# RazonIn4K/image-restoration-platform

Measured on AMD Instinct MI355X. Metric: restored images/sec @1024x1024 bs=8, higher is better.
Workload: dtype bf16; 1 GPU; 1024x1024 RGB u8, batch 8 per GPU: fused classifier scan + RestoreNet-v0 (43 convs, 779.9 GFLOP/image), seeded random-init weights; global_batch=8, parallelism=per-image data parallel x1, no collective, streams=1

## Files before the change

image_restoration_platform_amd/csrc/conv_pc.hip:

```cpp
#include "conv_mfma.hpp"
#include "conv_plan.hpp"
#include "gn_fold.hpp"
#include "persist.hpp"

#include <type_traits>

namespace ire {

namespace {

typedef __bf16 bf16x8_t __attribute__((ext_vector_type(8)));
typedef __bf16 bf16x2_t __attribute__((ext_vector_type(2)));
typedef float f32x2_t __attribute__((ext_vector_type(2)));
typedef float f32x16_t __attribute__((ext_vector_type(16)));
typedef unsigned u32x4_t __attribute__((ext_vector_type(4)));

#ifndef C3_RES_PRE
#define C3_RES_PRE -1
#endif
#ifndef C3_SCALAR
#define C3_SCALAR 1
#endif
#ifndef C3_PRIO
#define C3_PRIO 1
#endif
#ifndef C3_TEPI
#define C3_TEPI 1
#endif
#ifndef IRE_LD_ONCE32
#define IRE_LD_ONCE32 2
#endif
#ifndef C3_TEPI64
#define C3_TEPI64 1
#endif
#ifndef C3_PROD8
#define C3_PROD8 0
#endif
#ifndef C3_INTERIOR
#define C3_INTERIOR 0
#endif
#ifndef C3_ABL
#define C3_ABL 0
#endif
constexpr int C3_CONS = 512, C3_PROD = 256, C3_THREADS = C3_CONS + C3_PROD;
constexpr int pc_prod(int C, bool head) { return (C3_PROD8 && C == 32 && !head) ? 512 : 256; }
constexpr int C3_TH = 16, C3_TW = 32, C3_IH = C3_TH + 2, C3_IW = C3_TW + 2;
constexpr int C3_IN_CHUNKS = C3_IH * C3_IW * 4;
constexpr int C3_P_ITERS = (C3_IN_CHUNKS + C3_PROD - 1) / C3_PROD;
constexpr int C3_IN_BYTES = C3_P_ITERS * C3_PROD * 16;
template <int C> struct PcCfg {
    static constexpr int NT = C < 64 ? 32 : 64;
    static constexpr int NBLK = C / NT;
    static constexpr int NKC = C / 32;
    static constexpr int NTL = NT / 32;
    static constexpr int W_STAGE = 36 * NT * 16;
    static constexpr int W_STAGE_CHUNKS = 36 * NT;
    static constexpr int W_LDS = NKC * W_STAGE;
    static constexpr int W_OFF = 2 * C3_IN_BYTES;
    static constexpr int BIAS_OFF = W_OFF + W_LDS;
    static constexpr int NCC = NT / 8;
    static constexpr int RED_OFF = BIAS_OFF + C * 4;
    static constexpr int RED_HALF = 8 * NCC * 4;
    static constexpr int COEF_IMGS = pc_coef_imgs(C);
    static constexpr int COEF_OFF = RED_OFF + 2 * RED_HALF * 4;
    static constexpr int HEAD_OFF = COEF_OFF + COEF_IMGS * C * 2 * 4;
    static constexpr int PATCH_OFF = HEAD_OFF + (C == 32 ? 8 * 2 * 2 * 96 : 0);
    static constexpr int CNT_OFF = PATCH_OFF + (C == 32 ? 8 * 2048 : 0);
    static constexpr int LDS = CNT_OFF + (C == 64 ? 16 : 0);
    static_assert(LDS <= 160 * 1024, "LDS");
};

__device__ __forceinline__ unsigned c3_pack(float a, float b) {
    f32x2_t f = {a, b};
    return __builtin_bit_cast(unsigned, __builtin_convertvector(f, bf16x2_t));
}
__device__ __forceinline__ float c3_lo(unsigned u) { return __builtin_bit_cast(float, u << 16); }
__device__ __forceinline__ float c3_hi(unsigned u) { return __builtin_bit_cast(float, u & 0xffff0000u); }
template <int N> __device__ __forceinline__ float c3_ror_add(float v) {
    const int r = __builtin_amdgcn_update_dpp(0, __builtin_bit_cast(int, v), 0x120 + N, 0xf, 0xf, false);
    return v + __builtin_bit_cast(float, r);
}
__device__ __forceinline__ float c3_swap16_add(float v) {
    float x = v, y = v;
    asm volatile("v_nop\n\tv_nop\n\tv_permlane16_swap_b32 %0, %1" : "+v"(x), "+v"(y));
    return x + y;
}

__device__ __forceinline__ void c3_glds16(const void* gsrc, unsigned lds_dst_uniform) {
    unsigned keep;
    asm volatile("s_mov_b32 %0, m0\n\ts_mov_b32 m0, %2\n\ts_nop 0\n\tglobal_load_lds_dwordx4 %1, off\n\ts_mov_b32 m0, %0"
                 : "=&s"(keep) : "v"(gsrc), "s"(lds_dst_uniform) : "memory");
}
__device__ __forceinline__ void c3_barrier() { asm volatile("s_waitcnt lgkmcnt(0)\n\ts_barrier" ::: "memory"); }

template <int C, bool RESID, bool HEAD>
__global__ __launch_bounds__(C3_CONS + pc_prod(C, HEAD)) void conv_pc_kernel(ConvArgs a) {
    using K = PcCfg<C>;
    constexpr int PROD = pc_prod(C, HEAD), THREADS = C3_CONS + PROD;
    constexpr int P_ITERS = (C3_IN_CHUNKS + PROD - 1) / PROD;
    static_assert(P_ITERS * PROD * 16 == C3_IN_BYTES, "tile slots");
    constexpr int NKC = K::NKC, NTL = K::NTL, NCC = K::NCC, NT = K::NT;
    static_assert(!HEAD || C == 32, "the head is a C = 32 layer");
    __shared__ __attribute__((aligned(16))) unsigned char smem[K::LDS];
    const int tid = threadIdx.x;
    const int lane = tid & 63, wave = tid >> 6;
    const int r = lane & 31, h = lane >> 5;
    int stamp_item = 0;
    auto stamp = [&](int k) {
#ifdef IRE_PC_TICKS
        const unsigned long long t = __builtin_amdgcn_s_memtime();
        if (a.stamps && lane == 0 && (wave == 0 || wave == 8) && blockIdx.x < 8 && stamp_item < 64)
            a.stamps[(((size_t)blockIdx.x * 2 + (wave ? 1 : 0)) * 64 + stamp_item) * 10 + k] = t;
#else
        (void)k;
#endif
    };

    auto tl = [&](int slot) {
#ifdef IRE_W4_TL
        if (a.stamps && tid == 0) {
            a.stamps[(size_t)blockIdx.x * 32 + slot * 2] = __builtin_amdgcn_s_memrealtime();
            a.stamps[(size_t)blockIdx.x * 32 + slot * 2 + 1] = __builtin_amdgcn_s_memtime();
        }
#else
        (void)slot;
#endif
    };
    const int tiles_per_img = a.tiles_x * a.tiles_y;
    PersistCursor cursor(a.tiles_x, a.tiles_y, a.nimg, K::NBLK, NKC, (int)gridDim.x, (int)blockIdx.x, a.walk_rev != 0);
    const int n_items = cursor.my_items;
    if (n_items == 0) return;
    const int n_stages = n_items * NKC;
    tl(0);
    {
        const unsigned char* ws = reinterpret_cast<const unsigned char*>(a.w);
        const unsigned wl = (unsigned)(size_t)(__attribute__((address_space(3))) unsigned char*)smem + K::W_OFF;
        constexpr int PIECES = NKC * K::W_STAGE_CHUNKS / 64;
        static_assert((NKC * K::W_STAGE_CHUNKS) % 64 == 0, "whole wave-instructions");
        const int wv = __builtin_amdgcn_readfirstlane(wave);
        for (int p = wv; p < PIECES; p += THREADS / 64) c3_glds16(ws + ((size_t)p * 64 + lane) * 16, wl + p * 1024);
    }
    if (a.gn_stats) gn_fold(a, smem, cursor.first_img, cursor.last_img, 512, reinterpret_cast<float2*>(smem + K::COEF_OFF));
    tl(1);

    {
        if (tid < C) reinterpret_cast<float*>(smem + K::BIAS_OFF)[tid] = a.bias[tid];
        if constexpr (C == 64) { if (tid == 0) *reinterpret_cast<unsigned*>(smem + K::CNT_OFF) = 0u; }
        const int nim = cursor.last_img - cursor.first_img + 1;
        const float2* ab = a.ab + (size_t)cursor.first_img * C;
        float2* cd = reinterpret_cast<float2*>(smem + K::COEF_OFF);
        if (!a.gn_stats) for (int i = tid; i < nim * C; i += THREADS) cd[i] = ab[i];
    }
    asm volatile("s_waitcnt vmcnt(0)" ::: "memory");
    __syncthreads();
    tl(2);

    if (__builtin_amdgcn_readfirstlane(wave) >= 8) {
#if C3_PRIO
        if (C3_PRIO != 1 || C != 32 || HEAD) asm volatile("s_setprio %0" :: "n"(C3_PRIO));
#endif
        const int tp = tid - C3_CONS;
        const int c8 = tp & 3;
        int rel[P_ITERS], lds_off[P_ITERS];
        unsigned pyx[P_ITERS];
#pragma unroll
        for (int i = 0; i < P_ITERS; ++i) {
            const int q = tp + i * PROD;
            const int p = q >> 2;
            const int py = p / C3_IW, px = p - py * C3_IW;
            pyx[i] = ((unsigned)py << 8) | (unsigned)px;
            rel[i] = (py * a.Win + px) * (2 * C) + c8 * 16;
            lds_off[i] = (p * 4 + (c8 ^ ((p >> 2) & 3))) * 16;
        }
        uint4 R[P_ITERS];
        unsigned okbits = 0;
        float cA[8], cB[8];
        PersistStage ls = cursor.cur;
        auto load_chunk = [&](int i) __attribute__((always_inline)) {
            const PersistItem& lit = ls.it;
            const int oy1 = lit.ty * C3_TH - 1, ox1 = lit.tx * C3_TW - 1;
            const char* base = reinterpret_cast<const char*>(a.in0) + (size_t)lit.img * a.in_rows * a.Win * (2 * C) + ls.kc * 64;
            const __amdgpu_buffer_rsrc_t irsrc = __builtin_amdgcn_make_buffer_rsrc(const_cast<char*>(base), 0, a.in_rows * a.Win * (2 * C) - ls.kc * 64, 0x00020000);
            const int base_off = ((oy1 + a.in_row_off) * a.Win + ox1) * (2 * C);
            const int y_lo = max(a.iy_lo - oy1, 0), y_hi = min(a.iy_lo + a.iy_span - oy1, C3_IH);
            const int x_lo = max(-ox1, 0), x_hi = min(a.Win - ox1, C3_IW);
            const int py = (int)(pyx[i] >> 8), px = (int)(pyx[i] & 0xffu);
            const bool ok = (unsigned)(py - y_lo) < (unsigned)(y_hi - y_lo) && (unsigned)(px - x_lo) < (unsigned)(x_hi - x_lo);
            const unsigned off = ok ? (unsigned)(base_off + rel[i]) : 0xffffffffu;
            if constexpr (C3_ABL & 8) { R[i] = make_uint4(off, 0x3f803f80u, i, 0x3f803f80u); }
            else {
                const u32x4_t lv = __builtin_amdgcn_raw_buffer_load_b128(irsrc, off, 0, IRE_LD_IN);
                R[i] = make_uint4(lv.x, lv.y, lv.z, lv.w);
            }
            okbits = (okbits & ~(1u << i)) | (ok ? (1u << i) : 0u);
        };
        auto load_coeffs = [&](const PersistStage& st) __attribute__((always_inline)) {
            const float4* ab = reinterpret_cast<const float4*>(smem + K::COEF_OFF) + ((st.it.img - cursor.first_img) * C + st.kc * 32 + c8 * 8) / 2;
#pragma unroll
            for (int e = 0; e < 4; ++e) { const float4 v = ab[e]; cA[2 * e] = v.x; cB[2 * e] = v.y; cA[2 * e + 1] = v.z; cB[2 * e + 1] = v.w; }
        };
        auto transform_stage_v = [&](unsigned char* tile, auto interior_tag) __attribute__((always_inline)) {
            constexpr bool INTERIOR = decltype(interior_tag)::value;
            auto pair = [&](auto pp_tag) __attribute__((always_inline)) {
                constexpr int pp_ = decltype(pp_tag)::value, i = 2 * pp_;
                constexpr int NCH = i + 1 < P_ITERS ? 2 : 1;
                constexpr int NW = 4 * NCH, NV = 8 * NCH;
                constexpr int i1 = NCH == 2 ? i + 1 : i;
                const unsigned wds[8] = {R[i].x, R[i].y, R[i].z, R[i].w, R[i1].x, R[i1].y, R[i1].z, R[i1].w};
                unsigned o[8];
                if constexpr (C3_ABL & 1) {
#pragma unroll
                    for (int w = 0; w < NW; ++w) o[w] = wds[w];
                } else {
#if C3_SCALAR
                    float y[16], e[16];
#pragma unroll
                    for (int w = 0; w < NW; ++w) {
                        const int d = w & 3;
                        y[2 * w] = __builtin_fmaf(c3_lo(wds[w]), cA[2 * d], cB[2 * d]);
                        y[2 * w + 1] = __builtin_fmaf(c3_hi(wds[w]), cA[2 * d + 1], cB[2 * d + 1]);
                    }
#pragma unroll
                    for (int k = 0; k < NV; ++k) e[k] = y[k] * (-1.4426950408889634f);
                    __builtin_amdgcn_sched_barrier(0);
#pragma unroll
                    for (int k = 0; k < NV; ++k) e[k] = __builtin_amdgcn_exp2f(e[k]);
                    __builtin_amdgcn_sched_barrier(0);
#pragma unroll
                    for (int k = 0; k < NV; ++k) e[k] = e[k] + 1.0f;
                    __builtin_amdgcn_sched_barrier(0);
#pragma unroll
                    for (int k = 0; k < NV; ++k) e[k] = __builtin_amdgcn_rcpf(e[k]);
                    __builtin_amdgcn_sched_barrier(0);
#pragma unroll
                    for (int w = 0; w < NW; ++w) o[w] = c3_pack(y[2 * w] * e[2 * w], y[2 * w + 1] * e[2 * w + 1]);
#else
                    static_assert(NCH == 2, "the packed-f32 form handles whole pairs");
                    f32x2_t y[8], e[8];
#pragma unroll
                    for (int w = 0; w < 8; ++w) {
                        const int d = w & 3;
                        const f32x2_t x = {c3_lo(wds[w]), c3_hi(wds[w])};
                        const f32x2_t A = {cA[2 * d], cA[2 * d + 1]}, B = {cB[2 * d], cB[2 * d + 1]};
                        y[w] = __builtin_elementwise_fma(x, A, B);
                        e[w] = y[w] * (-1.4426950408889634f);
                    }
                    __builtin_amdgcn_sched_barrier(0);
#pragma unroll
                    for (int w = 0; w < 8; ++w) e[w] = f32x2_t{__builtin_amdgcn_exp2f(e[w].x), __builtin_amdgcn_exp2f(e[w].y)};
                    __builtin_amdgcn_sched_barrier(0);
#pragma unroll
                    for (int w = 0; w < 8; ++w) e[w] = e[w] + 1.0f;
                    __builtin_amdgcn_sched_barrier(0);
#pragma unroll
                    for (int w = 0; w < 8; ++w) e[w] = f32x2_t{__builtin_amdgcn_rcpf(e[w].x), __builtin_amdgcn_rcpf(e[w].y)};
                    __builtin_amdgcn_sched_barrier(0);
#pragma unroll
                    for (int w = 0; w < 8; ++w) { const f32x2_t sv = y[w] * e[w]; o[w] = c3_pack(sv.x, sv.y); }
#endif
                }
#pragma unroll
                for (int k = 0; k < NCH; ++k) {
                    uint4 ov = make_uint4(o[4 * k], o[4 * k + 1], o[4 * k + 2], o[4 * k + 3]);
                    if constexpr (!INTERIOR) {
                        const unsigned m = (okbits >> (i + k)) & 1u ? 0xffffffffu : 0u;
                        ov = make_uint4(o[4 * k] & m, o[4 * k + 1] & m, o[4 * k + 2] & m, o[4 * k + 3] & m);
                    }
                    *reinterpret_cast<uint4*>(tile + lds_off[i + k]) = ov;
                }
                load_chunk(i);
                if constexpr (NCH == 2) load_chunk(i + 1);
                __builtin_amdgcn_sched_barrier(0);
            };
            pair(std::integral_constant<int, 0>{}); pair(std::integral_constant<int, 1>{}); pair(std::integral_constant<int, 2>{});
            if constexpr (P_ITERS > 6) { pair(std::integral_constant<int, 3>{}); pair(std::integral_constant<int, 4>{}); }
        };
        unsigned past_last = 0u;
        {
            const int q = tp + (P_ITERS - 1) * PROD;
            past_last = (q >> 2) >= C3_IH * C3_IW ? (1u << (P_ITERS - 1)) : 0u;
        }
        auto transform_stage = [&](unsigned char* tile) __attribute__((always_inline)) {
            if constexpr (C3_INTERIOR) {
                if (__builtin_amdgcn_ballot_w64((okbits | past_last) != (1u << P_ITERS) - 1u) == 0) { transform_stage_v(tile, std::true_type{}); return; }
            }
            transform_stage_v(tile, std::false_type{});
        };
#pragma unroll
        for (int i = 0; i < P_ITERS; ++i) load_chunk(i);
        load_coeffs(ls);
        ls = cursor.next();
        transform_stage(smem);
        c3_barrier();
        for (int t = 0; t < n_stages; ++t) {
            stamp_item = t / NKC;
            stamp(3 * (t % NKC) + 0);
            load_coeffs(ls);
            ls = cursor.next();
            transform_stage(smem + ((t + 1) & 1) * C3_IN_BYTES);
            stamp(3 * (t % NKC) + 1);
            c3_barrier();
            stamp(3 * (t % NKC) + 2);
        }
        return;
    }

    int a_off[2][9];
#pragma unroll
    for (int m = 0; m < 2; ++m)
#pragma unroll
        for (int tap = 0; tap < 9; ++tap) {
            const int ky = tap / 3, kx = tap - ky * 3;
            const int p = (wave * 2 + m + ky) * C3_IW + r + kx;
            a_off[m][tap] = (p * 4 + (h ^ ((p >> 2) & 3))) * 16;
        }
    const unsigned char* wb = smem + K::W_OFF + (h * NT + r) * 16;
    const float* bias_lds = reinterpret_cast<const float*>(smem + K::BIAS_OFF);
    f32x16_t bias_acc;
    if constexpr (C == 32) {
#pragma unroll
        for (int i = 0; i < 16; ++i) bias_acc[i] = bias_lds[16 * (i >> 3) + 8 * h + (i & 7)];
    }
    float* red_base = reinterpret_cast<float*>(smem + K::RED_OFF);
    int st_img = -1, st_tile = 0, st_nb = 0, st_par = 0, red_par = 0;
    auto flush_stats = [&]() {
        if (HEAD || st_img < 0) return;
        constexpr int G = C / 8, NGL = NT / G, CPG = G / 8;
        if (tid < NGL) {
            const float* red = red_base + st_par * K::RED_HALF;
            float s = 0.f, q = 0.f;
#pragma unroll
            for (int w = 0; w < 8; ++w) {
                if constexpr (C == 32) {
                    const float* d = red + (w * NCC + (tid >> 1)) * 4 + 2 * (tid & 1);
                    s += d[0]; q += d[1];
                } else {
#pragma unroll
                    for (int k = 0; k < CPG; ++k) {
                        const float* d = red + (w * NCC + tid * CPG + k) * 4;
                        s += d[0] + d[2]; q += d[1] + d[3];
                    }
                }
            }
            float* st = a.stats + (((size_t)st_img * tiles_per_img + st_tile) * 8 + (st_nb * NT) / G + tid) * 2;
            st[0] = s; st[1] = q;
        }
        st_img = -1;
    };

    f32x16_t acc[2][NTL];
    uint4 erv[2 * NTL][2];
    constexpr int RES_WANT = C3_RES_PRE >= 0 ? C3_RES_PRE : (C == 64 ? 1 : 2);
    constexpr int RES_PRE = RES_WANT < 2 * NTL ? RES_WANT : 2 * NTL;
    unsigned eoffs[2];
    bool einb[2];
    constexpr bool TEPI = C3_TEPI && C == 32 && !HEAD;
    constexpr bool TEPI64 = C3_TEPI64 && C == 64 && !HEAD;
    unsigned toffs[2];
    bool trow[2];
    int tcol = 0;
    unsigned hin[2] = {0u, 0u};
    size_t hoff[2] = {0, 0};
    bool hok[2] = {false, false};
    PersistStage cs = cursor.cur;
    int stage_no = 0;
    c3_barrier();
    for (int t = 0; t < n_items; ++t) {
        const PersistItem it = cs.it;
        stamp_item = t;
        stamp(0);
        flush_stats();
        {
            const int oyb = it.ty * C3_TH + wave * 2, ox = it.tx * C3_TW + r;
            const bool colok = ox < a.Wout;
            const int oxc = min(ox, a.Wout - 1);
#pragma unroll
            for (int m = 0; m < 2; ++m) {
                const int oy = oyb + m;
                einb[m] = colok && oy < a.Hout;
                eoffs[m] = ((unsigned)((min(oy, a.Hout - 1) * a.Wout + oxc) * C + it.nb * NT) << 1) + (unsigned)(h * 16);
            }
            if constexpr (TEPI || TEPI64) {
                constexpr int LPP = C / 8;
                tcol = it.tx * C3_TW + lane / LPP;
#pragma unroll
                for (int m = 0; m < 2; ++m) {
                    const int oy = oyb + m;
                    trow[m] = oy < a.Hout;
                    toffs[m] = ((unsigned)((min(oy, a.Hout - 1) * a.Wout + tcol) * C + 8 * (lane % LPP)) << 1);
                }
            }
            if constexpr (RESID && TEPI64 && !(C3_ABL & 64)) {
                char* rbase = const_cast<char*>(reinterpret_cast<const char*>(a.resid)) + (size_t)it.img * a.Hout * a.Wout * (2 * C);
                const __amdgpu_buffer_rsrc_t rrsrc = __builtin_amdgcn_make_buffer_rsrc(rbase, 0, a.Hout * a.Wout * (2 * C), 0x00020000);
#pragma unroll
                for (int m = 0; m < 2; ++m)
#pragma unroll
                    for (int k = 0; k < RES_PRE; ++k) {
                        const bool ok = trow[m] && tcol + 8 * k < a.Wout;
                        const u32x4_t v = __builtin_amdgcn_raw_buffer_load_b128(rrsrc, ok ? toffs[m] + (unsigned)(8 * k * 2 * C) : 0xffffffffu, 0, IRE_LD_ONCE32);
                        erv[k][m] = make_uint4(v.x, v.y, v.z, v.w);
                    }
            } else
            if constexpr (RESID && TEPI && !(C3_ABL & 64)) {
                char* rbase = const_cast<char*>(reinterpret_cast<const char*>(a.resid)) + (size_t)it.img * a.Hout * a.Wout * (2 * C);
                const __amdgpu_buffer_rsrc_t rrsrc = __builtin_amdgcn_make_buffer_rsrc(rbase, 0, a.Hout * a.Wout * (2 * C), 0x00020000);
#pragma unroll
                for (int m = 0; m < 2; ++m)
#pragma unroll
                    for (int k = 0; k < 2; ++k) {
                        const bool ok = trow[m] && tcol + 16 * k < a.Wout;
                        const u32x4_t v = __builtin_amdgcn_raw_buffer_load_b128(rrsrc, ok ? toffs[m] + (unsigned)(16 * k * 2 * C) : 0xffffffffu, 0, IRE_LD_ONCE);
                        erv[k][m] = make_uint4(v.x, v.y, v.z, v.w);
                    }
            } else if constexpr (RESID && (C3_ABL & 64)) {
#pragma unroll
                for (int g = 0; g < 2 * NTL; ++g)
#pragma unroll
                    for (int m = 0; m < 2; ++m) erv[g][m] = make_uint4(eoffs[m], g, 0x3f803f80u, m);
            } else if constexpr (RESID) {
                const char* rbase = reinterpret_cast<const char*>(a.resid) + (size_t)it.img * a.Hout * a.Wout * (2 * C);
#pragma unroll
                for (int m = 0; m < 2; ++m)
#pragma unroll
                    for (int g = 0; g < RES_PRE; ++g) erv[g][m] = *reinterpret_cast<const uint4*>(rbase + eoffs[m] + (unsigned)(g * 32));
            }
            if constexpr (HEAD) {
                const int vbytes = 3 * min(C3_TW, a.Wout - it.tx * C3_TW);
#pragma unroll
                for (int m = 0; m < 2; ++m) {
                    const int oy = oyb + m;
                    hok[m] = oy < a.Hout && 4 * lane < vbytes;
                    hoff[m] = (((size_t)it.img * a.Hout + min(oy, a.Hout - 1)) * a.Wout + it.tx * C3_TW) * 3 + 4 * (size_t)min(lane, 23);
                    hin[m] = hok[m] ? *reinterpret_cast<const unsigned*>(a.u8_in + hoff[m]) : 0u;
                }
            }
        }
        if constexpr (C != 32) {
#pragma unroll
            for (int j = 0; j < NTL; ++j)
#pragma unroll
                for (int q = 0; q < 4; ++q) {
                    const float4 bv = *reinterpret_cast<const float4*>(bias_lds + it.nb * NT + j * 32 + 16 * (q >> 1) + 8 * h + 4 * (q & 1));
#pragma unroll
                    for (int m = 0; m < 2; ++m) { acc[m][j][4 * q + 0] = bv.x; acc[m][j][4 * q + 1] = bv.y; acc[m][j][4 * q + 2] = bv.z; acc[m][j][4 * q + 3] = bv.w; }
                }
        }
#pragma unroll NKC <= 2 ? NKC : 1
        for (int kc = 0; kc < NKC; ++kc) {
          auto stage_body = [&](auto par_tag) __attribute__((always_inline)) {
            constexpr int PAR = decltype(par_tag)::value;
            const int par = PAR >= 0 ? PAR : (stage_no & 1);
            const unsigned char* ib = smem + par * C3_IN_BYTES;
            const unsigned char* wk = wb + kc * K::W_STAGE;
            bf16x8_t af[2][2], bf[2][NTL];
            auto read_k = [&](int g, bf16x8_t (&pa)[2], bf16x8_t (&pw)[NTL]) __attribute__((always_inline)) {
                const int tap = g >> 1, cp = g & 1;
#pragma unroll
                for (int m = 0; m < 2; ++m) pa[m] = __builtin_bit_cast(bf16x8_t, *reinterpret_cast<const uint4*>(ib + (a_off[m][tap] ^ (cp << 5))));
#pragma unroll
                for (int j = 0; j < NTL; ++j) pw[j] = __builtin_bit_cast(bf16x8_t, *reinterpret_cast<const uint4*>(wk + ((tap * 4 + 2 * cp) * NT + j * 32) * 16));
            };
            read_k(0, af[0], bf[0]);
            if constexpr (!(C3_ABL & 4))
#pragma unroll
            for (int g = 0; g < 18; ++g) {
                if (g + 1 < 18) read_k(g + 1, af[(g + 1) & 1], bf[(g + 1) & 1]);
                __builtin_amdgcn_sched_barrier(0);
#pragma unroll
                for (int m = 0; m < 2; ++m)
#pragma unroll
                    for (int j = 0; j < NTL; ++j) {
                        if constexpr (C == 32) acc[m][j] = __builtin_amdgcn_mfma_f32_32x32x16_bf16(bf[g & 1][j], af[g & 1][m], (kc == 0 && g == 0) ? bias_acc : acc[m][j], 0, 0, 0);
                        else acc[m][j] = __builtin_amdgcn_mfma_f32_32x32x16_bf16(bf[g & 1][j], af[g & 1][m], acc[m][j], 0, 0, 0);
                    }
                __builtin_amdgcn_sched_barrier(0);
            }
          };
            if constexpr (NKC == 1 && HEAD) { if (stage_no & 1) stage_body(std::integral_constant<int, 1>{}); else stage_body(std::integral_constant<int, 0>{}); }
            else if constexpr (NKC == 2) { if (kc & 1) stage_body(std::integral_constant<int, 1>{}); else stage_body(std::integral_constant<int, 0>{}); }
            else stage_body(std::integral_constant<int, -1>{});
            ++stage_no;
            stamp(kc == 0 ? 1 : 3);
            if (kc + 1 < NKC) { cs = cursor.next(); c3_barrier(); stamp(2); }
        }
        if constexpr (RESID && TEPI64 && RES_PRE < 2 * NTL) {
            char* rbase = const_cast<char*>(reinterpret_cast<const char*>(a.resid)) + (size_t)it.img * a.Hout * a.Wout * (2 * C);
            const __amdgpu_buffer_rsrc_t rrsrc = __builtin_amdgcn_make_buffer_rsrc(rbase, 0, a.Hout * a.Wout * (2 * C), 0x00020000);
#pragma unroll
            for (int m = 0; m < 2; ++m)
#pragma unroll
                for (int k = RES_PRE; k < 2 * NTL; ++k) {
                    const bool ok = trow[m] && tcol + 8 * k < a.Wout;
                    const u32x4_t v = __builtin_amdgcn_raw_buffer_load_b128(rrsrc, ok ? toffs[m] + (unsigned)(8 * k * 2 * C) : 0xffffffffu, 0, 0);
                    erv[k][m] = make_uint4(v.x, v.y, v.z, v.w);
                }
        } else if constexpr (RESID && RES_PRE < 2 * NTL) {
            const char* rbase = reinterpret_cast<const char*>(a.resid) + (size_t)it.img * a.Hout * a.Wout * (2 * C);
#pragma unroll
            for (int m = 0; m < 2; ++m)
#pragma unroll
                for (int g = RES_PRE; g < 2 * NTL; ++g) erv[g][m] = *reinterpret_cast<const uint4*>(rbase + eoffs[m] + (unsigned)(g * 32));
        }
        if constexpr (HEAD) {
            unsigned char* hp = smem + K::HEAD_OFF + wave * (2 * 2 * 96);
#pragma unroll
            for (int m = 0; m < 2; ++m)
                if (lane < 24) *reinterpret_cast<unsigned*>(hp + m * 96 + 4 * lane) = hin[m];
#pragma unroll
            for (int m = 0; m < 2; ++m) {
                if (h == 0) {
#pragma unroll
                    for (int c = 0; c < 3; ++c) {
                        float vv = (float)hp[m * 96 + 3 * r + c] + acc[m][0][c];
                        vv = fminf(fmaxf(vv, 0.f), 255.f);
                        hp[192 + m * 96 + 3 * r + c] = (unsigned char)(int)floorf(vv + 0.5f);
                    }
                }
            }
#pragma unroll
            for (int m = 0; m < 2; ++m)
                if (hok[m]) *reinterpret_cast<unsigned*>(a.u8_out + hoff[m]) = *reinterpret_cast<const unsigned*>(hp + 192 + m * 96 + 4 * min(lane, 23));
        } else if constexpr (C3_ABL & 2) {
#pragma unroll
            for (int m = 0; m < 2; ++m)
#pragma unroll
                for (int j = 0; j < NTL; ++j) asm volatile("" :: "v"(acc[m][j]));
        } else if constexpr (TEPI64) {
            char* obase = reinterpret_cast<char*>(a.out) + (size_t)it.img * a.Hout * a.Wout * (2 * C);
            const __amdgpu_buffer_rsrc_t orsrc = __builtin_amdgcn_make_buffer_rsrc(obase, 0, a.Hout * a.Wout * (2 * C), 0x00020000);
            const bf16x2_t ones = __builtin_bit_cast(bf16x2_t, 0x3f803f80u);
            float* redw = red_base + red_par * K::RED_HALF;
            {
                volatile unsigned* cnt = reinterpret_cast<volatile unsigned*>(smem + K::CNT_OFF);
                asm volatile("s_waitcnt lgkmcnt(0)" ::: "memory");
                if (lane == 0) __hip_atomic_fetch_add(const_cast<unsigned*>(cnt), 1u, __ATOMIC_RELAXED, __HIP_MEMORY_SCOPE_WORKGROUP);
                const unsigned target = 8u * (unsigned)(t + 1);
                while ((unsigned)__builtin_amdgcn_readfirstlane((int)*cnt) < target) __builtin_amdgcn_s_sleep(1);
            }
            unsigned char* patch = smem + C3_IN_BYTES + wave * 4096;
            const int wsw = r & 7;
            const int pq = lane >> 3, cq = lane & 7;
            float sA = 0.f, qA = 0.f;
#pragma unroll
            for (int half = 0; half < 2; ++half)
#pragma unroll
            for (int m = 0; m < 2; ++m) {
#pragma unroll
                for (int g = 0; g < 2 * NTL; ++g) {
                    const f32x16_t& c = acc[m][g >> 1];
                    const int pp = g & 1;
                    const u32x4_t wv = {c3_pack(c[8 * pp + 0], c[8 * pp + 1]), c3_pack(c[8 * pp + 2], c[8 * pp + 3]),
                                        c3_pack(c[8 * pp + 4], c[8 * pp + 5]), c3_pack(c[8 * pp + 6], c[8 * pp + 7])};
                    *reinterpret_cast<u32x4_t*>(patch + r * 128 + (((2 * g + h) ^ wsw) << 4)) = wv;
                }
#pragma unroll
                for (int k = 2 * half; k < 2 * half + 2; ++k) {
                    const int p = pq + 8 * k;
                    const u32x4_t v = *reinterpret_cast<const u32x4_t*>(patch + p * 128 + ((cq ^ (p & 7)) << 4));
                    unsigned w[4] = {v.x, v.y, v.z, v.w};
                    if constexpr (RESID) {
                        const uint4 rr = erv[k][m];
                        const unsigned rw[4] = {rr.x, rr.y, rr.z, rr.w};
#pragma unroll
                        for (int d = 0; d < 4; ++d) w[d] = c3_pack(c3_lo(w[d]) + c3_lo(rw[d]), c3_hi(w[d]) + c3_hi(rw[d]));
                    }
                    const bool ok = trow[m] && tcol + 8 * k < a.Wout;
                    const float mf = ok ? 1.f : 0.f;
                    float ts0 = 0.f, tq0 = 0.f;
                    if constexpr (!(C3_ABL & 32))
#pragma unroll
                    for (int d = 0; d < 4; ++d) {
                        const bf16x2_t bv = __builtin_bit_cast(bf16x2_t, w[d]);
                        ts0 = __builtin_amdgcn_fdot2_f32_bf16(bv, ones, ts0, false); tq0 = __builtin_amdgcn_fdot2_f32_bf16(bv, bv, tq0, false);
                    }
                    sA = __builtin_fmaf(ts0, mf, sA); qA = __builtin_fmaf(tq0, mf, qA);
                    const u32x4_t o4 = {w[0], w[1], w[2], w[3]};
                    if constexpr (C3_ABL & 16) asm volatile("" :: "v"(o4));
                    else __builtin_amdgcn_raw_buffer_store_b128(o4, orsrc, ok ? toffs[m] + (unsigned)(8 * k * 2 * C) : 0xffffffffu, 0, IRE_ST_LINE);
                }
            }
            if constexpr (!(C3_ABL & 32)) {
                float t2[2] = {sA, qA};
#pragma unroll
                for (int k = 0; k < 2; ++k) t2[k] = c3_ror_add<8>(t2[k]);
#pragma unroll
                for (int k = 0; k < 2; ++k) t2[k] = c3_swap16_add(t2[k]);
#pragma unroll
                for (int k = 0; k < 2; ++k) { float x = t2[k], y = t2[k]; asm volatile("v_nop\n\tv_nop\n\tv_permlane32_swap_b32 %0, %1" : "+v"(x), "+v"(y)); t2[k] = x + y; }
                if (lane < 8) *reinterpret_cast<float4*>(redw + (wave * NCC + lane) * 4) = make_float4(t2[0], t2[1], 0.f, 0.f);
            }
            st_img = it.img; st_tile = it.tile; st_nb = it.nb; st_par = red_par; red_par ^= 1;
        } else if constexpr (TEPI) {
            char* obase = reinterpret_cast<char*>(a.out) + (size_t)it.img * a.Hout * a.Wout * (2 * C);
            const __amdgpu_buffer_rsrc_t orsrc = __builtin_amdgcn_make_buffer_rsrc(obase, 0, a.Hout * a.Wout * (2 * C), 0x00020000);
            const bf16x2_t ones = __builtin_bit_cast(bf16x2_t, 0x3f803f80u);
            float* redw = red_base + red_par * K::RED_HALF;
            unsigned char* patch = smem + K::PATCH_OFF + wave * 2048;
            const int wsw = (r >> 1) & 3;
            const int pq = lane >> 2, cq = lane & 3;
            float sA = 0.f, qA = 0.f, sB = 0.f, qB = 0.f;
#pragma unroll
            for (int m = 0; m < 2; ++m) {
                const f32x16_t& c = acc[m][0];
#pragma unroll
                for (int pp = 0; pp < 2; ++pp) {
                    const u32x4_t wv = {c3_pack(c[8 * pp + 0], c[8 * pp + 1]), c3_pack(c[8 * pp + 2], c[8 * pp + 3]),
                                        c3_pack(c[8 * pp + 4], c[8 * pp + 5]), c3_pack(c[8 * pp + 6], c[8 * pp + 7])};
                    *reinterpret_cast<u32x4_t*>(patch + r * 64 + (((2 * pp + h) ^ wsw) << 4)) = wv;
                }
#pragma unroll
                for (int k = 0; k < 2; ++k) {
                    const int p = pq + 16 * k;
                    const u32x4_t v = *reinterpret_cast<const u32x4_t*>(patch + p * 64 + ((cq ^ ((p >> 1) & 3)) << 4));
                    unsigned w[4] = {v.x, v.y, v.z, v.w};
                    if constexpr (RESID) {
                        const uint4 rr = erv[k][m];
                        const unsigned rw[4] = {rr.x, rr.y, rr.z, rr.w};
#pragma unroll
                        for (int d = 0; d < 4; ++d) w[d] = c3_pack(c3_lo(w[d]) + c3_lo(rw[d]), c3_hi(w[d]) + c3_hi(rw[d]));
                    }
                    const bool ok = trow[m] && tcol + 16 * k < a.Wout;
                    const float mf = ok ? 1.f : 0.f;
                    float ts0 = 0.f, tq0 = 0.f, ts1 = 0.f, tq1 = 0.f;
                    if constexpr (!(C3_ABL & 32))
#pragma unroll
                    for (int d = 0; d < 4; ++d) {
                        const bf16x2_t bv = __builtin_bit_cast(bf16x2_t, w[d]);
                        if (d < 2) { ts0 = __builtin_amdgcn_fdot2_f32_bf16(bv, ones, ts0, false); tq0 = __builtin_amdgcn_fdot2_f32_bf16(bv, bv, tq0, false); }
                        else { ts1 = __builtin_amdgcn_fdot2_f32_bf16(bv, ones, ts1, false); tq1 = __builtin_amdgcn_fdot2_f32_bf16(bv, bv, tq1, false); }
                    }
                    sA = __builtin_fmaf(ts0, mf, sA); qA = __builtin_fmaf(tq0, mf, qA);
                    sB = __builtin_fmaf(ts1, mf, sB); qB = __builtin_fmaf(tq1, mf, qB);
                    const u32x4_t o4 = {w[0], w[1], w[2], w[3]};
                    if constexpr (C3_ABL & 16) asm volatile("" :: "v"(o4));
                    else __builtin_amdgcn_raw_buffer_store_b128(o4, orsrc, ok ? toffs[m] + (unsigned)(16 * k * 2 * C) : 0xffffffffu, 0, IRE_ST_LINE);
                }
            }
            if constexpr (!(C3_ABL & 32)) {
                float t4[4] = {sA, qA, sB, qB};
#pragma unroll
                for (int k = 0; k < 4; ++k) t4[k] = c3_ror_add<4>(t4[k]);
#pragma unroll
                for (int k = 0; k < 4; ++k) t4[k] = c3_ror_add<8>(t4[k]);
#pragma unroll
                for (int k = 0; k < 4; ++k) t4[k] = c3_swap16_add(t4[k]);
#pragma unroll
                for (int k = 0; k < 4; ++k) { float x = t4[k], y = t4[k]; asm volatile("v_nop\n\tv_nop\n\tv_permlane32_swap_b32 %0, %1" : "+v"(x), "+v"(y)); t4[k] = x + y; }
                if (lane < 4) *reinterpret_cast<float4*>(redw + (wave * NCC + lane) * 4) = make_float4(t4[0], t4[1], t4[2], t4[3]);
            }
            st_img = it.img; st_tile = it.tile; st_nb = it.nb; st_par = red_par; red_par ^= 1;
        } else {
            char* obase = reinterpret_cast<char*>(a.out) + (size_t)it.img * a.Hout * a.Wout * (2 * C);
            const __amdgpu_buffer_rsrc_t orsrc = __builtin_amdgcn_make_buffer_rsrc(obase, 0, a.Hout * a.Wout * (2 * C), 0x00020000);
            const bf16x2_t ones = __builtin_bit_cast(bf16x2_t, 0x3f803f80u);
            float* redw = red_base + red_par * K::RED_HALF;
            const float mf[2] = {einb[0] ? 1.f : 0.f, einb[1] ? 1.f : 0.f};
            float vs[4], vq[4];
#pragma unroll
            for (int j = 0; j < NTL; ++j)
#pragma unroll
            for (int pp = 0; pp < 2; ++pp) {
                const int g = 2 * j + pp;
                float sA = 0.f, qA = 0.f, sB = 0.f, qB = 0.f;
#pragma unroll
                for (int m = 0; m < 2; ++m) {
                    const f32x16_t& c = acc[m][j];
                    unsigned w[4] = {c3_pack(c[8 * pp + 0], c[8 * pp + 1]), c3_pack(c[8 * pp + 2], c[8 * pp + 3]),
                                     c3_pack(c[8 * pp + 4], c[8 * pp + 5]), c3_pack(c[8 * pp + 6], c[8 * pp + 7])};
                    if constexpr (RESID) {
                        const uint4 rr = erv[g][m];
                        const unsigned rw[4] = {rr.x, rr.y, rr.z, rr.w};
#pragma unroll
                        for (int d = 0; d < 4; ++d) w[d] = c3_pack(c3_lo(w[d]) + c3_lo(rw[d]), c3_hi(w[d]) + c3_hi(rw[d]));
                    }
                    float ts0 = 0.f, tq0 = 0.f, ts1 = 0.f, tq1 = 0.f;
                    if constexpr (!(C3_ABL & 32))
#pragma unroll
                    for (int d = 0; d < 4; ++d) {
                        const bf16x2_t wv = __builtin_bit_cast(bf16x2_t, w[d]);
                        if (d < 2 || C != 32) { ts0 = __builtin_amdgcn_fdot2_f32_bf16(wv, ones, ts0, false); tq0 = __builtin_amdgcn_fdot2_f32_bf16(wv, wv, tq0, false); }
                        else { ts1 = __builtin_amdgcn_fdot2_f32_bf16(wv, ones, ts1, false); tq1 = __builtin_amdgcn_fdot2_f32_bf16(wv, wv, tq1, false); }
                    }
                    sA = __builtin_fmaf(ts0, mf[m], sA); qA = __builtin_fmaf(tq0, mf[m], qA);
                    if constexpr (C == 32) { sB = __builtin_fmaf(ts1, mf[m], sB); qB = __builtin_fmaf(tq1, mf[m], qB); }
                    const u32x4_t wv4 = {w[0], w[1], w[2], w[3]};
                    if constexpr (C3_ABL & 16) asm volatile("" :: "v"(wv4));
                    else __builtin_amdgcn_raw_buffer_store_b128(wv4, orsrc, einb[m] ? eoffs[m] + (unsigned)(g * 32) : 0xffffffffu, 0, IRE_ST_PART);
                }
                if constexpr (C == 32) { vs[2 * pp] = sA; vq[2 * pp] = qA; vs[2 * pp + 1] = sB; vq[2 * pp + 1] = qB; }
                else { vs[g] = sA; vq[g] = qA; }
            }
            if constexpr (!(C3_ABL & 32)) {
                const bool b0 = lane & 1, b1 = lane & 2;
                auto xch = [&](float keep, float give, auto ctrl_tag) __attribute__((always_inline)) -> float {
                    const int gg = __builtin_amdgcn_update_dpp(0, __builtin_bit_cast(int, give), decltype(ctrl_tag)::value, 0xf, 0xf, false);
                    return keep + __builtin_bit_cast(float, gg);
                };
                float u[4], t2[2];
#pragma unroll
                for (int k = 0; k < 4; ++k) u[k] = xch(b0 ? vq[k] : vs[k], b0 ? vs[k] : vq[k], std::integral_constant<int, 0xb1>{});
#pragma unroll
                for (int k = 0; k < 2; ++k) t2[k] = xch(b1 ? u[2 + k] : u[k], b1 ? u[k] : u[2 + k], std::integral_constant<int, 0x4e>{});
                t2[0] = c3_ror_add<4>(t2[0]); t2[1] = c3_ror_add<4>(t2[1]);
                t2[0] = c3_ror_add<8>(t2[0]); t2[1] = c3_ror_add<8>(t2[1]);
                t2[0] = c3_swap16_add(t2[0]); t2[1] = c3_swap16_add(t2[1]);
                if ((lane & 28) == 0) {
                    if constexpr (C == 32) {
                        float* d = redw + (wave * NCC + (b1 ? 2 : 0) + h) * 4 + (b0 ? 1 : 0);
                        d[0] = t2[0]; d[2] = t2[1];
                    } else {
                        float* d = redw + (wave * NCC + (b1 ? 4 : 0) + h) * 4 + (b0 ? 1 : 0);
                        d[0] = t2[0]; d[8] = t2[1];
                        d[2] = 0.f; d[10] = 0.f;
                    }
                }
            }
            st_img = it.img; st_tile = it.tile; st_nb = it.nb; st_par = red_par; red_par ^= 1;
        }
        stamp(NKC == 1 ? 3 : 4);
        cs = cursor.next();
        c3_barrier();
        stamp(5);
        tl(3 + (t < 8 ? t : 8));
    }
    flush_stats();
    tl(12);
}

}

void conv_pc_launch(bool resid, bool head, const ConvArgs& a, hipStream_t stream) {
    const int C = a.cout;
    if ((C != 32 && C != 64) || a.cin0 != C || a.nkc != C / 32 || a.nblocks != 1 || !a.ab)
        fail(IRE_ERR_INTERNAL, "internal: conv_pc arguments");
    if (head ? (C != 32 || !a.u8_in || !a.u8_out) : !a.stats) fail(IRE_ERR_INTERNAL, "internal: conv_pc arguments");
    const int items = a.tiles_x * a.tiles_y * a.nimg * a.nblocks;
    const int cus = persistent_grid_cus();
    if (!coef_table_fits(pc_coef_imgs(C), (long long)a.tiles_x * a.tiles_y, a.nimg, cus)) fail(IRE_ERR_INTERNAL, "internal: conv_pc batch");
    const int grid = items < cus ? items : cus;
#define PC_GO(CC, RS, HD) hipLaunchKernelGGL((conv_pc_kernel<CC, RS, HD>), dim3(grid), dim3(C3_CONS + pc_prod(CC, HD)), 0, stream, a)
    if (head) PC_GO(32, false, true);
    else if (C == 32) { if (resid) PC_GO(32, true, false); else PC_GO(32, false, false); }
    else { if (resid) PC_GO(64, true, false); else PC_GO(64, false, false); }
#undef PC_GO
    IRE_HIP(hipGetLastError());
}

}
```

Measured before the change: 1116 images/sec.

## Hoist halo border masking out of the producer loop with parked LDS writes

Drops the per-chunk bounds test and the AND-masking of transformed values in the producer waves of the persistent conv kernel. The padding window is now computed once per stage. Only when that window changes is a zero mask recomputed; padded chunks are then redirected to a spare 'park' LDS slot and their real slots are zeroed. Each double buffer remembers which window it was last cleaned for, so repeated border zeroing is skipped. This cuts producer VALU and branch work, at the cost of extra state, some unmasked out-of-window loads, and correctness that depends on the park area and the clean-tracking logic.

```diff
diff --git a/image_restoration_platform_amd/csrc/conv_pc.hip b/image_restoration_platform_amd/csrc/conv_pc.hip
--- a/image_restoration_platform_amd/csrc/conv_pc.hip
+++ b/image_restoration_platform_amd/csrc/conv_pc.hip
@@ -1,6 +1,7 @@
 #include "conv_mfma.hpp"
 #include "conv_plan.hpp"
 #include "gn_fold.hpp"
+#include "pc_border.hpp"
 #include "persist.hpp"
 
 #include <type_traits>
@@ -36,15 +37,12 @@
 #ifndef C3_PROD8
 #define C3_PROD8 0
 #endif
-#ifndef C3_INTERIOR
-#define C3_INTERIOR 0
-#endif
 #ifndef C3_ABL
 #define C3_ABL 0
 #endif
 constexpr int C3_CONS = 512, C3_PROD = 256, C3_THREADS = C3_CONS + C3_PROD;
 constexpr int pc_prod(int C, bool head) { return (C3_PROD8 && C == 32 && !head) ? 512 : 256; }
-constexpr int C3_TH = 16, C3_TW = 32, C3_IH = C3_TH + 2, C3_IW = C3_TW + 2;
+constexpr int C3_TH = PC_TILE_H, C3_TW = PC_TILE_W, C3_IH = PC_HALO_H, C3_IW = PC_HALO_W;
 constexpr int C3_IN_CHUNKS = C3_IH * C3_IW * 4;
 constexpr int C3_P_ITERS = (C3_IN_CHUNKS + C3_PROD - 1) / C3_PROD;
 constexpr int C3_IN_BYTES = C3_P_ITERS * C3_PROD * 16;
@@ -162,18 +160,13 @@
         const int tp = tid - C3_CONS;
         const int c8 = tp & 3;
         int rel[P_ITERS], lds_off[P_ITERS];
-        unsigned pyx[P_ITERS];
 #pragma unroll
         for (int i = 0; i < P_ITERS; ++i) {
-            const int q = tp + i * PROD;
-            const int p = q >> 2;
-            const int py = p / C3_IW, px = p - py * C3_IW;
-            pyx[i] = ((unsigned)py << 8) | (unsigned)px;
-            rel[i] = (py * a.Win + px) * (2 * C) + c8 * 16;
-            lds_off[i] = (p * 4 + (c8 ^ ((p >> 2) & 3))) * 16;
+            const PcPixel hp = pc_chunk_pixel(tp, i, PROD);
+            rel[i] = (hp.py * a.Win + hp.px) * (2 * C) + c8 * 16;
+            lds_off[i] = pc_slot_off(tp + i * PROD);
         }
         uint4 R[P_ITERS];
-        unsigned okbits = 0;
         float cA[8], cB[8];
         PersistStage ls = cursor.cur;
         auto load_chunk = [&](int i) __attribute__((always_inline)) {
@@ -182,25 +175,22 @@
             const char* base = reinterpret_cast<const char*>(a.in0) + (size_t)lit.img * a.in_rows * a.Win * (2 * C) + ls.kc * 64;
             const __amdgpu_buffer_rsrc_t irsrc = __builtin_amdgcn_make_buffer_rsrc(const_cast<char*>(base), 0, a.in_rows * a.Win * (2 * C) - ls.kc * 64, 0x00020000);
             const int base_off = ((oy1 + a.in_row_off) * a.Win + ox1) * (2 * C);
-            const int y_lo = max(a.iy_lo - oy1, 0), y_hi = min(a.iy_lo + a.iy_span - oy1, C3_IH);
-            const int x_lo = max(-ox1, 0), x_hi = min(a.Win - ox1, C3_IW);
-            const int py = (int)(pyx[i] >> 8), px = (int)(pyx[i] & 0xffu);
-            const bool ok = (unsigned)(py - y_lo) < (unsigned)(y_hi - y_lo) && (unsigned)(px - x_lo) < (unsigned)(x_hi - x_lo);
-            const unsigned off = ok ? (unsigned)(base_off + rel[i]) : 0xffffffffu;
+            const unsigned off = (unsigned)(base_off + rel[i]);
             if constexpr (C3_ABL & 8) { R[i] = make_uint4(off, 0x3f803f80u, i, 0x3f803f80u); }
             else {
                 const u32x4_t lv = __builtin_amdgcn_raw_buffer_load_b128(irsrc, off, 0, IRE_LD_IN);
                 R[i] = make_uint4(lv.x, lv.y, lv.z, lv.w);
             }
-            okbits = (okbits & ~(1u << i)) | (ok ? (1u << i) : 0u);
         };
         auto load_coeffs = [&](const PersistStage& st) __attribute__((always_inline)) {
             const float4* ab = reinterpret_cast<const float4*>(smem + K::COEF_OFF) + ((st.it.img - cursor.first_img) * C + st.kc * 32 + c8 * 8) / 2;
 #pragma unroll
             for (int e = 0; e < 4; ++e) { const float4 v = ab[e]; cA[2 * e] = v.x; cB[2 * e] = v.y; cA[2 * e + 1] = v.z; cB[2 * e + 1] = v.w; }
         };
-        auto transform_stage_v = [&](unsigned char* tile, auto interior_tag) __attribute__((always_inline)) {
-            constexpr bool INTERIOR = decltype(interior_tag)::value;
+        int lds_eff[P_ITERS];
+#pragma unroll
+        for (int i = 0; i < P_ITERS; ++i) lds_eff[i] = lds_off[i];
+        auto transform_stage = [&](unsigned char* tile) __attribute__((always_inline)) {
             auto pair = [&](auto pp_tag) __attribute__((always_inline)) {
                 constexpr int pp_ = decltype(pp_tag)::value, i = 2 * pp_;
                 constexpr int NCH = i + 1 < P_ITERS ? 2 : 1;
@@ -260,14 +250,8 @@
 #endif
                 }
 #pragma unroll
-                for (int k = 0; k < NCH; ++k) {
-                    uint4 ov = make_uint4(o[4 * k], o[4 * k + 1], o[4 * k + 2], o[4 * k + 3]);
-                    if constexpr (!INTERIOR) {
-                        const unsigned m = (okbits >> (i + k)) & 1u ? 0xffffffffu : 0u;
-                        ov = make_uint4(o[4 * k] & m, o[4 * k + 1] & m, o[4 * k + 2] & m, o[4 * k + 3] & m);
-                    }
-                    *reinterpret_cast<uint4*>(tile + lds_off[i + k]) = ov;
-                }
+                for (int k = 0; k < NCH; ++k)
+                    *reinterpret_cast<uint4*>(tile + lds_eff[i + k]) = make_uint4(o[4 * k], o[4 * k + 1], o[4 * k + 2], o[4 * k + 3]);
                 load_chunk(i);
                 if constexpr (NCH == 2) load_chunk(i + 1);
                 __builtin_amdgcn_sched_barrier(0);
@@ -275,29 +259,45 @@
             pair(std::integral_constant<int, 0>{}); pair(std::integral_constant<int, 1>{}); pair(std::integral_constant<int, 2>{});
             if constexpr (P_ITERS > 6) { pair(std::integral_constant<int, 3>{}); pair(std::integral_constant<int, 4>{}); }
         };
-        unsigned past_last = 0u;
-        {
-            const int q = tp + (P_ITERS - 1) * PROD;
-            past_last = (q >> 2) >= C3_IH * C3_IW ? (1u << (P_ITERS - 1)) : 0u;
-        }
-        auto transform_stage = [&](unsigned char* tile) __attribute__((always_inline)) {
-            if constexpr (C3_INTERIOR) {
-                if (__builtin_amdgcn_ballot_w64((okbits | past_last) != (1u << P_ITERS) - 1u) == 0) { transform_stage_v(tile, std::true_type{}); return; }
-            }
-            transform_stage_v(tile, std::false_type{});
+        constexpr bool TILE1_REUSED = C3_TEPI64 && C == 64 && !HEAD;
+        unsigned zm = 0u, eff_key = pc_window_key(PcWindow{0, C3_IH, 0, C3_IW}), clean0 = 0u, clean1 = 0u;
+        auto produce = [&](int b) __attribute__((always_inline)) {
+            unsigned char* tile = smem + b * C3_IN_BYTES;
+            load_coeffs(ls);
+            const PcWindow win = pc_window(ls.it.ty, ls.it.tx, a.iy_lo, a.iy_span, a.Win);
+            const unsigned key = pc_window_key(win);
+            ls = cursor.next();
+            if constexpr (!(C3_ABL & 128)) {
+                if (key != eff_key) {
+                    int tq = tp;
+                    asm volatile("" : "+v"(tq));
+                    zm = pc_zero_mask(win, tq, PROD, P_ITERS);
+                    const int park = pc_park_off(tq);
+#pragma unroll
+                    for (int i = 0; i < P_ITERS; ++i) lds_eff[i] = (zm & (1u << i)) ? park : lds_off[i];
+                    eff_key = key;
+                }
+            }
+            transform_stage(tile);
+            if constexpr (!(C3_ABL & 128)) {
+                const unsigned had = b ? clean1 : clean0;
+                if (!pc_interior(win) && (had != key || (TILE1_REUSED && b))) {
+#pragma unroll
+                    for (int i = 0; i < P_ITERS; ++i)
+                        if (zm & (1u << i)) *reinterpret_cast<uint4*>(tile + lds_off[i]) = make_uint4(0u, 0u, 0u, 0u);
+                }
+                clean0 = b ? clean0 : key;
+                clean1 = b ? key : clean1;
+            }
         };
 #pragma unroll
         for (int i = 0; i < P_ITERS; ++i) load_chunk(i);
-        load_coeffs(ls);
-        ls = cursor.next();
-        transform_stage(smem);
+        produce(0);
         c3_barrier();
         for (int t = 0; t < n_stages; ++t) {
             stamp_item = t / NKC;
             stamp(3 * (t % NKC) + 0);
-            load_coeffs(ls);
-            ls = cursor.next();
-            transform_stage(smem + ((t + 1) & 1) * C3_IN_BYTES);
+            produce((t + 1) & 1);
             stamp(3 * (t % NKC) + 1);
             c3_barrier();
             stamp(3 * (t % NKC) + 2);
diff --git a/image_restoration_platform_amd/csrc/pc_border.hpp b/image_restoration_platform_amd/csrc/pc_border.hpp
--- /dev/null
+++ b/image_restoration_platform_amd/csrc/pc_border.hpp
@@ -0,0 +1,48 @@
+#pragma once
+
+#include "persist.hpp"
+
+namespace ire {
+
+constexpr int PC_TILE_H = 16, PC_TILE_W = 32, PC_HALO_H = PC_TILE_H + 2, PC_HALO_W = PC_TILE_W + 2;
+
+struct PcWindow { int y_lo, y_hi, x_lo, x_hi; };
+struct PcPixel { int py, px; };
+
+IRE_HD PcWindow pc_window(int ty, int tx, int iy_lo, int iy_span, int Win) {
+    const int oy1 = ty * PC_TILE_H - 1, ox1 = tx * PC_TILE_W - 1;
+    PcWindow w;
+    w.y_lo = iy_lo - oy1 > 0 ? iy_lo - oy1 : 0;
+    w.y_hi = iy_lo + iy_span - oy1 < PC_HALO_H ? iy_lo + iy_span - oy1 : PC_HALO_H;
+    w.x_lo = -ox1 > 0 ? -ox1 : 0;
+    w.x_hi = Win - ox1 < PC_HALO_W ? Win - ox1 : PC_HALO_W;
+    return w;
+}
+
+IRE_HD bool pc_interior(const PcWindow& w) { return w.y_lo == 0 && w.y_hi == PC_HALO_H && w.x_lo == 0 && w.x_hi == PC_HALO_W; }
+
+IRE_HD PcPixel pc_chunk_pixel(int tp, int i, int prod) {
+    const unsigned p = (unsigned)(tp + i * prod) >> 2;
+    PcPixel r;
+    r.py = (int)(p / (unsigned)PC_HALO_W);
+    r.px = (int)(p - (unsigned)r.py * (unsigned)PC_HALO_W);
+    return r;
+}
+
+IRE_HD bool pc_chunk_padded(const PcWindow& w, const PcPixel& p) {
+    return p.py < PC_HALO_H && !((unsigned)(p.py - w.y_lo) < (unsigned)(w.y_hi - w.y_lo) && (unsigned)(p.px - w.x_lo) < (unsigned)(w.x_hi - w.x_lo));
+}
+
+IRE_HD unsigned pc_zero_mask(const PcWindow& w, int tp, int prod, int iters) {
+    unsigned z = 0u;
+    for (int i = 0; i < iters; ++i) z |= pc_chunk_padded(w, pc_chunk_pixel(tp, i, prod)) ? 1u << i : 0u;
+    return z;
+}
+IRE_HD unsigned pc_window_key(const PcWindow& w) { return (unsigned)w.y_lo | (unsigned)w.y_hi << 8 | (unsigned)w.x_lo << 16 | (unsigned)w.x_hi << 24; }
+IRE_HD int pc_slot_off(int q) {
+    const int p = q >> 2, c8 = q & 3;
+    return (p * 4 + (c8 ^ ((p >> 2) & 3))) * 16;
+}
+IRE_HD int pc_park_off(int tp) { return (PC_HALO_H * PC_HALO_W * 4 + (tp & 63)) * 16; }
+
+}
```

Measured after the change: 1123 images/sec (median of 6 runs). No clear change (+0.7%).
